# Nahuel-M/StereoVisionArray

Measured on NVIDIA B200. Metric: MDE/s, higher is better.
Workload: dtype u16

## Files before the change

stereovisionarray_b200/csrc/k_ad.cu:

```cuda
#include "sva_common.cuh"

struct AdPairs {
    int32_t alpha[SVA_MAX_PAIRS], beta[SVA_MAX_PAIRS], base[SVA_MAX_PAIRS], g[SVA_MAX_PAIRS];
    unsigned long long line_off[SVA_MAX_PAIRS];
    int32_t n;
};

__global__ void k_build_line_image(const uint8_t* __restrict__ img, int W, int H, size_t img_pitch, uint8_t* __restrict__ line,
                                   int a, int b, int u, int v, int cmin, int tmin, int pad, int pitch) {
    int x = blockIdx.x * blockDim.x + threadIdx.x, y = blockIdx.y;
    if (x >= W) return;
    int c = b * x - a * y - cmin, t = u * x + v * y - tmin + pad;
    line[(size_t)c * pitch + t] = img[(size_t)y * img_pitch + x];
}

__device__ __forceinline__ void ad_accumulate(uint32_t diff, uint32_t& even, uint32_t& odd) {
    even += diff & 0x00FF00FFu;
    odd += __byte_perm(diff, 0, 0x4341);
}

__device__ __forceinline__ void ad_gather8(const uint8_t* __restrict__ L, int off, int g, uint32_t& b0, uint32_t& b1) {
    const uint32_t* wp = (const uint32_t*)(L + (off & ~3));
    const int sh = (off & 3) * 8;
    if (g == 1) {
        uint32_t w0 = __ldg(wp), w1 = __ldg(wp + 1), w2 = __ldg(wp + 2);
        b0 = __funnelshift_r(w0, w1, sh);
        b1 = __funnelshift_r(w1, w2, sh);
    } else if (g == 2) {
        uint32_t w0 = __ldg(wp), w1 = __ldg(wp + 1), w2 = __ldg(wp + 2), w3 = __ldg(wp + 3), w4 = __ldg(wp + 4);
        uint32_t a0 = __funnelshift_r(w0, w1, sh), a1 = __funnelshift_r(w1, w2, sh);
        uint32_t a2 = __funnelshift_r(w2, w3, sh), a3 = __funnelshift_r(w3, w4, sh);
        b0 = __byte_perm(a0, a1, 0x6420);
        b1 = __byte_perm(a2, a3, 0x6420);
    } else {
        const uint8_t* q = L + off;
        b0 = q[0] | (q[g] << 8) | (q[2 * g] << 16) | ((uint32_t)q[3 * g] << 24);
        b1 = q[4 * g] | (q[5 * g] << 8) | (q[6 * g] << 16) | ((uint32_t)q[7 * g] << 24);
    }
}

__global__ void __launch_bounds__(256)
k_ad_planar(const uint8_t* __restrict__ ref, size_t ref_pitch, const uint8_t* __restrict__ lines, AdPairs P, int W, int H, int D, int dmin,
            uint32_t* __restrict__ AP, int wp, int padl, int padt) {
    const int nch = D >> 3, per_group = 2 * nch;
    const long long id = (long long)blockIdx.x * blockDim.x + threadIdx.x;
    const long long G = id / per_group;
    const int tl = (int)(id - G * per_group);
    const int half = tl / nch, chunk = tl - half * nch;
    const int tiles_x = (W + 7) >> 3;
    const long long tile = G >> 3;
    const int ty = (int)(tile / tiles_x), tx = (int)(tile - (long long)ty * tiles_x);
    const int y = ty * 8 + (int)(G & 7);
    if (y >= H) return;
    const int x0 = tx * 8 + 4 * half;
    int xc[4];
    uint32_t r4[4];
#pragma unroll
    for (int i = 0; i < 4; i++) {
        xc[i] = min(x0 + i, W - 1);
        r4[i] = (uint32_t)ref[(size_t)y * ref_pitch + xc[i]] * 0x01010101u;
    }
    const int delta0 = dmin + 8 * chunk;
    uint32_t e0[4], o0[4], e1[4], o1[4];
#pragma unroll
    for (int i = 0; i < 4; i++) { e0[i] = 0; o0[i] = 0; e1[i] = 0; o1[i] = 0; }
    for (int k = 0; k < P.n; k++) {
        const uint8_t* L = lines + P.line_off[k];
        const int g = P.g[k], alpha = P.alpha[k];
        const int offb = P.base[k] + y * P.beta[k] + g * delta0;
#pragma unroll
        for (int i = 0; i < 4; i++) {
            uint32_t b0, b1;
            ad_gather8(L, offb + xc[i] * alpha, g, b0, b1);
            ad_accumulate(__vabsdiffu4(b0, r4[i]), e0[i], o0[i]);
            ad_accumulate(__vabsdiffu4(b1, r4[i]), e1[i], o1[i]);
        }
    }
    uint32_t w[4][4];
#pragma unroll
    for (int i = 0; i < 4; i++) {
        const bool in = x0 + i < W;
        w[i][0] = in ? __byte_perm(e0[i], o0[i], 0x5410) : 0u;
        w[i][1] = in ? __byte_perm(e0[i], o0[i], 0x7632) : 0u;
        w[i][2] = in ? __byte_perm(e1[i], o1[i], 0x5410) : 0u;
        w[i][3] = in ? __byte_perm(e1[i], o1[i], 0x7632) : 0u;
    }
    uint32_t* out = AP + ((size_t)(y + padt) * (D >> 1) + 4 * chunk) * wp + padl + x0;
#pragma unroll
    for (int j = 0; j < 4; j++) *reinterpret_cast<uint4*>(out + (size_t)j * wp) = make_uint4(w[0][j], w[1][j], w[2][j], w[3][j]);
}

__global__ void k_ap_unpack(const uint32_t* __restrict__ AP, int W, int H, int dph, int wp, int padl, int padt, uint32_t* __restrict__ out) {
    const int x = blockIdx.x * blockDim.x + threadIdx.x, y = blockIdx.y;
    if (x >= W) return;
    for (int dp = 0; dp < dph; dp++) out[((size_t)y * W + x) * dph + dp] = AP[((size_t)(y + padt) * dph + dp) * wp + padl + x];
}

static void ext_gcd(int a, int b, int& g, int& u, int& v) {
    if (b == 0) { g = a < 0 ? -a : a; u = a < 0 ? -1 : 1; v = 0; return; }
    int g1, u1, v1;
    ext_gcd(b, a % b, g1, u1, v1);
    g = g1; u = v1; v = u1 - (a / b) * v1;
}

int sva_build_line_images(sva_ctx* ctx) {
    const sva_params& p = ctx->prm;
    const int W = p.width, H = p.height, dmax = p.min_disp + p.num_disp - 1;
    size_t total = 0;
    for (int k = 0; k < p.n_pairs; k++) {
        PairGeom& G = ctx->geom[k];
        int gx = p.pair_gx[k], gy = p.pair_gy[k];
        if (gx == 0 && gy == 0) return ctx->fail(SVA_ERR_BAD_ARG, "pair offset (0,0)");
        int g, u, v, one;
        ext_gcd(-gx, -gy, g, u, v);
        int a = -gx / g, b = -gy / g;
        ext_gcd(a, b, one, u, v);
        G.g = g; G.a = a; G.b = b; G.u = u; G.v = v;
        int cs[4] = {0, b * (W - 1), -a * (H - 1), b * (W - 1) - a * (H - 1)};
// ... 18 lines not shown
        const PairGeom& G = ctx->geom[k];
        dim3 grid(div_up(W, 256), H);
        LaunchScope ls(ctx, "k_build_line_image");
        k_build_line_image<<<grid, 256, 0, ctx->stream>>>(ctx->other_imgs.as<uint8_t>() + (size_t)k * W * H, W, H, (size_t)W,
                                                         ctx->lines.as<uint8_t>() + G.offset, G.a, G.b, G.u, G.v, G.cmin, G.tmin, G.pad, G.pitch);
    }
    SVA_CUDA_OK(ctx, cudaGetLastError());
    return SVA_OK;
}

int sva_ap_prepare(sva_ctx* ctx) {
    const sva_params& p = ctx->prm;
    const int W = p.width, H = p.height, D = p.num_disp, k = p.win_half;
    ApGeom g;
    const int kk = (k + 3) & ~3;
    g.padl = kk; g.padt = k;
    g.txo = (256 - kk - k + 1) & ~3;
    g.strips = div_up(W, g.txo);
    g.wp = g.txo * (g.strips - 1) + 256;
    const int need = kk + ((W + 7) & ~7);
    if (g.wp < need) g.wp = need;
    g.wp = (g.wp + 7) & ~7;
    g.hp = H + 2 * k;
    g.row_words = (size_t)(D >> 1) * g.wp;
    g.words = (size_t)g.hp * g.row_words;
    SVA_TRY(ctx->reserve(ctx->AP, g.words * 4));
    ctx->ap = g;
    uint64_t key = (uint64_t)(uintptr_t)ctx->AP.p;
    key = key * 1000003u + (uint64_t)W; key = key * 1000003u + (uint64_t)H; key = key * 1000003u + (uint64_t)D; key = key * 1000003u + (uint64_t)k;
    if (key != ctx->ap_zero_key) {
        SVA_CUDA_OK(ctx, cudaMemsetAsync(ctx->AP.p, 0, g.words * 4, ctx->stream));
        ctx->ap_zero_key = key;
    }
    return SVA_OK;
}

int sva_ap_unpack(sva_ctx* ctx) {
    const sva_params& p = ctx->prm;
    const int W = p.width, H = p.height, D = p.num_disp;
    SVA_TRY(ctx->reserve(ctx->A, (size_t)W * H * D * sizeof(uint16_t)));
    LaunchScope ls(ctx, "k_ap_unpack");
    k_ap_unpack<<<dim3(div_up(W, 128), H), 128, 0, ctx->stream>>>(ctx->AP.as<uint32_t>(), W, H, D >> 1, ctx->ap.wp, ctx->ap.padl, ctx->ap.padt, ctx->A.as<uint32_t>());
    SVA_CUDA_OK(ctx, cudaGetLastError());
    return SVA_OK;
}

int sva_run_ad(sva_ctx* ctx) {
    const sva_params& p = ctx->prm;
    const int W = p.width, H = p.height, D = p.num_disp;
    SVA_TRY(sva_ap_prepare(ctx));
    AdPairs P;
    P.n = ctx->pair_end - ctx->pair_begin;
    for (int i = 0; i < P.n; i++) {
        const PairGeom& G = ctx->geom[ctx->pair_begin + i];
        P.alpha[i] = G.alpha; P.beta[i] = G.beta; P.base[i] = G.base; P.g[i] = G.g; P.line_off[i] = G.offset;
    }
    {
        LaunchScope ls(ctx, "k_ad_planar");
        const long long threads = (long long)div_up(W, 8) * div_up(H, 8) * 8 * (2 * (D >> 3));
        k_ad_planar<<<(unsigned)((threads + 255) / 256), 256, 0, ctx->stream>>>(ctx->ref_img.as<uint8_t>(), (size_t)W, ctx->lines.as<uint8_t>(), P, W, H, D, p.min_disp,
                                                                             ctx->AP.as<uint32_t>(), ctx->ap.wp, ctx->ap.padl, ctx->ap.padt);
    }
    SVA_CUDA_OK(ctx, cudaGetLastError());
    ctx->have_ad = true;
    return SVA_OK;
}
```

stereovisionarray_b200/csrc/k_ad2.cu:

```cuda
#include <algorithm>
#include <cstdlib>

#include "sva_common.cuh"

#define AD2_TH 8
#define AD2_TW 128
#define AD2_DR 32
#define AD2_THREADS 512
#define AD2_MAXG 2
#define AD2_SMEM_BUDGET (110 * 1024)

__host__ __device__ constexpr int ad2_sp(int agx, int dr = AD2_DR) { return dr == 32 ? (agx == 0 ? 160 : (agx == 1 ? 192 : 224)) : (agx == 0 ? 160 : (agx == 1 ? 176 : 192)); }
__host__ __device__ constexpr int ad2_rows(int agy, int th, int dr = AD2_DR) { return th + (dr - 1) * agy; }
#define AD2_TH_MAX 48

struct Ad2Params {
    const uint8_t* ref;
    const uint8_t* imgs;
    size_t img_bytes;
    int rp, pp, padx, pady;
    int W, H, D, dmin;
    uint32_t* AP;
    int wp, padl, padt;
    int n;
    int8_t gx[SVA_MAX_PAIRS], gy[SVA_MAX_PAIRS], phi[SVA_MAX_PAIRS];
    uint8_t img[SVA_MAX_PAIRS];
    int ngroups;
    uint8_t gbeg[SVA_MAX_PAIRS + 1];
    int row0, row1;
    int th;
    uint32_t one;
};

template <int GX, int GY, bool FMA = false, int DR = AD2_DR>
__device__ __forceinline__ void ad2_pair(const uint32_t* __restrict__ bp, const uint32_t r, uint32_t (&ax)[16], uint32_t (&ao)[16], const uint32_t one = 1u) {
    constexpr int SP = ad2_sp(GX < 0 ? -GX : GX, DR);
#pragma unroll
    for (int i = 0; i < 16; i++) {
        const int boff = -i * (GY * SP + GX);
        const int al = ((boff % 4) + 4) % 4;
        const int w0 = (boff - al) / 4;
        uint32_t w = bp[w0];
        if (al != 0) w = __funnelshift_r(w, bp[w0 + 1], 8 * al);
        const uint32_t ad = __vabsdiffu4(w, r);
        if (FMA) {
            ax[i] = ad * one + ax[i];
// ... 67 lines not shown
        sh.src[k] = q.imgs + (size_t)q.img[k] * q.img_bytes + (size_t)(q.pady + ylo) * q.pp + c0;
        sh.geo[k] = make_int2(soff, rows);
    }
    __syncthreads();
    const uint32_t smem_base = (uint32_t)__cvta_generic_to_shared(smem);
    for (int k = kb; k < ke; k++) {
        const int2 geo = sh.geo[k];
        const int sp = sh.pk[k].y, cpr = sp >> 4, n = geo.y * cpr;
        const uint32_t inv = 65536u / (uint32_t)cpr + 1u;
        const uint8_t* src0 = sh.src[k];
        const uint32_t dst0 = smem_base + geo.x;
        for (int c = t; c < n; c += AD2_THREADS) {
            const int rr = (int)(((uint32_t)c * inv) >> 16), cc = (c - rr * cpr) << 4;
            asm volatile("cp.async.cg.shared.global [%0], [%1], 16;" ::"r"(dst0 + rr * sp + cc), "l"(src0 + (size_t)rr * q.pp + cc) : "memory");
        }
    }
    asm volatile("cp.async.commit_group;" ::: "memory");
    asm volatile("cp.async.wait_group 0;" ::: "memory");
    __syncthreads();
}

__device__ __forceinline__ void ad2_store(const Ad2Params& q, const int y, const int x, const int d0, const uint32_t (&ax)[16], const uint32_t (&ao)[16]) {
    if (y >= q.H || x >= q.W || d0 >= q.D) return;
    uint32_t* out = q.AP + ((size_t)(y + q.padt) * (q.D >> 1) + (d0 >> 1)) * q.wp + q.padl + x;
    uint32_t me = 0xFFFFFFFFu, mo = 0xFFFFFFFFu;
    if (x + 3 >= q.W) {
        me = (x + 2 < q.W) ? 0xFFFFFFFFu : 0x0000FFFFu;
        mo = (x + 1 < q.W) ? 0x0000FFFFu : 0u;
    }
    const int np = min(8, (q.D - d0) >> 1);
#pragma unroll
    for (int i = 0; i < 8; i++) {
        const uint32_t o0 = ao[2 * i] & mo, o1 = ao[2 * i + 1] & mo;
        const uint32_t e0 = (ax[2 * i] - (ao[2 * i] << 8)) & me, e1 = (ax[2 * i + 1] - (ao[2 * i + 1] << 8)) & me;
        const uint4 v = make_uint4(__byte_perm(e0, e1, 0x5410), __byte_perm(o0, o1, 0x5410), __byte_perm(e0, e1, 0x7632), __byte_perm(o0, o1, 0x7632));
        if (i < np) *reinterpret_cast<uint4*>(out + (size_t)i * q.wp) = v;
    }
}

template <bool MULTI>
__global__ void __launch_bounds__(AD2_THREADS, 2)
k_ad_tile(const Ad2Params q) {
    extern __shared__ __align__(16) unsigned char ad2_smem[];
    __shared__ Ad2Shared sh;
    const int t = threadIdx.x;
    const int quad = t & 31, sub = (t >> 5) & 1, yl = t >> 6;
    const int x0 = blockIdx.x * AD2_TW, y0 = q.row0 + blockIdx.y * q.th, da = blockIdx.z * AD2_DR;
    const int x = x0 + 4 * quad, d0 = da + 16 * sub;
    uint32_t ax[16], ao[16];
    if (MULTI) {
        const int y = y0 + yl;
        const uint32_t r = *reinterpret_cast<const uint32_t*>(q.ref + (size_t)y * q.rp + x);
#pragma unroll
        for (int i = 0; i < 16; i++) { ax[i] = 0; ao[i] = 0; }
        for (int g = 0; g < q.ngroups; g++) {
            const int kb = q.gbeg[g], ke = q.gbeg[g + 1];
            if (g > 0) __syncthreads();
            ad2_stage(q, sh, ad2_smem, kb, ke, x0, y0, da);
#pragma unroll 1
// ... 121 lines not shown
        SVA_CUDA_OK(ctx, cudaMemsetAsync(ctx->pad_ref.p, 0, (size_t)g.rp * g.ref_rows, ctx->stream));
        ctx->ad2_zero_key = key;
    }
    ctx->ad2 = g;
    return SVA_OK;
}

uint8_t* sva_ad2_view_origin(sva_ctx* ctx, int k) {
    const sva_params& p = ctx->prm;
    const int phi = ((p.pair_gx[k] * p.min_disp) % 4 + 4) % 4;
    return ctx->pad_imgs.as<uint8_t>() + (size_t)k * ctx->ad2.img_bytes + (size_t)ctx->ad2.pady * ctx->ad2.pp + ctx->ad2.padx + phi;
}

int sva_ap_prepare(sva_ctx* ctx);

int sva_run_ad2(sva_ctx* ctx) {
    const sva_params& p = ctx->prm;
    const int W = p.width, H = p.height, D = p.num_disp;
    SVA_TRY(sva_ap_prepare(ctx));
    Ad2Params q{};
    q.ref = ctx->pad_ref.as<uint8_t>(); q.imgs = ctx->pad_imgs.as<uint8_t>(); q.img_bytes = ctx->ad2.img_bytes;
    q.rp = ctx->ad2.rp; q.pp = ctx->ad2.pp; q.padx = ctx->ad2.padx; q.pady = ctx->ad2.pady;
    q.W = W; q.H = H; q.D = D; q.dmin = p.min_disp;
    q.AP = ctx->AP.as<uint32_t>(); q.wp = ctx->ap.wp; q.padl = ctx->ap.padl; q.padt = ctx->ap.padt;
    q.n = ctx->pair_end - ctx->pair_begin;
    q.one = 1u;
    for (int i = 0; i < q.n; i++) {
        const int k = ctx->pair_begin + i;
        q.gx[i] = (int8_t)p.pair_gx[k]; q.gy[i] = (int8_t)p.pair_gy[k]; q.img[i] = (uint8_t)k;
        q.phi[i] = (int8_t)(((p.pair_gx[k] * p.min_disp) % 4 + 4) % 4);
    }
    if (q.n == 0) {
        SVA_CUDA_OK(ctx, cudaMemsetAsync(ctx->AP.p, 0, ctx->ap.words * 4, ctx->stream));
        ctx->have_ad = true;
        return SVA_OK;
    }
    int ya = 0, yb = H;
    if (ctx->win_rows > 0) { ya = std::max(0, ctx->win_y0 - p.win_half); yb = std::min(H, ctx->win_y0 + ctx->win_rows + p.win_half); }
    q.row0 = ya / AD2_TH * AD2_TH; q.row1 = yb;
    void (*kern)(Ad2Params) = nullptr;
    int dr = AD2_DR;
    if (ctx->tune_ad_set) {
        if (ad2_set_matches<Ad2Set3x3>(q)) { kern = k_ad_tile_set<Ad2Set3x3>; dr = Ad2Set3x3::dr; }
        else if (ad2_set_matches<Ad2SetPair>(q)) { kern = k_ad_tile_set<Ad2SetPair>; dr = Ad2SetPair::dr; }
        else if (ad2_set_matches<Ad2Set4x4>(q)) { kern = k_ad_tile_set<Ad2Set4x4>; dr = Ad2Set4x4::dr; }
    }
    const int rstep = dr == 32 ? 8 : 16;
// ... 40 lines not shown
```

stereovisionarray_b200/csrc/k_box.cu:

```cuda
#include <algorithm>

#include "sva_common.cuh"

#define BOX_THREADS 256
#define BOX_DP 16
#define BOX_CG 16
#define BOX_MAX_BAND 512

struct BoxParams {
    const uint16_t* A;
    void* out;
    int W, H, D, k, dmin, shift, cap;
    int gxp, gxn, gyp, gyn;
    int band_rows, txo;
    int apply_validity;
};

__device__ __forceinline__ int axis_limit(int pos, int dim, int k, int gp, int gn) {
    if (pos < k || pos >= dim - k) return -1;
    int lim = 0x7FFFFFFF;
    if (gp > 0) lim = min(lim, (pos - k) / gp);
    if (gn > 0) lim = min(lim, (dim - k - pos) / gn);
    return lim;
}
// ... 142 lines not shown
    if (bands < 1) bands = 1;
    if (div_up(H, bands) > BOX_MAX_BAND) bands = div_up(H, BOX_MAX_BAND);
    q.band_rows = div_up(H, bands);
    bands = div_up(H, q.band_rows);
    dim3 grid(strips, dch, bands);
    LaunchScope ls(ctx, raw ? "k_box_cost_raw" : "k_box_cost");
    cudaError_t e;
    if (wide) e = raw ? box_launch<8, true>(q, grid, ctx->stream) : box_launch<8, false>(q, grid, ctx->stream);
    else e = raw ? box_launch<4, true>(q, grid, ctx->stream) : box_launch<4, false>(q, grid, ctx->stream);
    SVA_CUDA_OK(ctx, e);
    return SVA_OK;
}

#define BXP_WARPS 8
#define BXP_TCOLS 48
#define BXP_OPITCH 260
#define BXP_MAX_BAND 1024

struct BoxPParams {
    const uint32_t* AP;
    uint16_t* C;
    int W, H, D, k, kk, dmin, shift, cap;
    int gxp, gxn, gyp, gyn;
    int band_rows, txo, wp;
    int l2hint;
    int chunk;
    long long row_words;
    int ry0, ry1;
};

__global__ void __launch_bounds__(256, 2)
k_box_planar(BoxPParams q) {
    __shared__ __align__(16) uint32_t s_out[2][BXP_WARPS][BXP_OPITCH];
    __shared__ __align__(8) unsigned long long s_bar[2];
    __shared__ uint2 s_T[BXP_WARPS][8 * BXP_TCOLS];
    __shared__ int s_limy[BXP_MAX_BAND];
    const int t = threadIdx.x, lane = t & 31, warp = t >> 5;
    const int W = q.W, H = q.H, D = q.D, k = q.k;
    const int dpc = min((int)blockIdx.y * BXP_WARPS + warp, (D >> 1) - 1);
    const int d = 2 * dpc;
    const int xs = blockIdx.x * q.txo - q.kk;
    const int y0 = q.ry0 + blockIdx.z * q.band_rows, y1 = min(q.ry1, y0 + q.band_rows);
    for (int i = t; i < y1 - y0; i += 256) s_limy[i] = axis_limit(y0 + i, H, k, q.gyp, q.gyn);

    int thr[8], thrmin = 0x7FFFFFFF;
#pragma unroll
    for (int j = 0; j < 8; j++) {
        thr[j] = axis_limit(xs + lane * 8 + j, W, k, q.gxp, q.gxn) - q.dmin - d;
        thrmin = min(thrmin, thr[j]);
    }
    uint2* tbl = &s_T[warp][8 + lane];
    if (lane == 0) tbl[0] = make_uint2(0u, 0u);
    const uint32_t bar0 = (uint32_t)__cvta_generic_to_shared(&s_bar[0]);
    if (t == 0) {
        asm volatile("mbarrier.init.shared::cta.b64 [%0], %1;" ::"r"(bar0), "r"(BXP_WARPS) : "memory");
        asm volatile("mbarrier.init.shared::cta.b64 [%0], %1;" ::"r"(bar0 + 8), "r"(BXP_WARPS) : "memory");
    }
    int offh[8], offl[8];
#pragma unroll
    for (int j = 0; j < 8; j++) {
        offh[j] = ((j + k) & 7) * BXP_TCOLS + ((j + k) >> 3);
        offl[j] = ((j - k) & 7) * BXP_TCOLS + ((j - k) >> 3);
    }
    __syncthreads();

    const uint32_t* pz = q.AP + (size_t)dpc * q.wp + (size_t)blockIdx.x * q.txo + lane * 8;
    const uint32_t* pe = pz + (size_t)y0 * q.row_words;
    const long long back = 2LL * k * q.row_words;
    const int N = (y1 - y0) + 2 * k - 1;
    uint32_t F[8], Vh[8];
#pragma unroll
    for (int j = 0; j < 8; j++) { F[j] = 0; Vh[j] = 0; }

    const int hf = t & 1;
    const bool half_ok = (int)blockIdx.y * 16 + 8 * hf < D;
    const int xl0 = t >> 1, xl1 = xl0 + 128;
    const bool st0 = half_ok && xl0 >= q.kk && xl0 < q.kk + q.txo && xs + xl0 < W;
    const bool st1 = half_ok && xl1 >= q.kk && xl1 < q.kk + q.txo && xs + xl1 < W;
    uint16_t* po = q.C + ((size_t)y0 * W + (xs + xl0)) * D + blockIdx.y * 16 + 8 * hf;
    const size_t orow = (size_t)W * D;
    const uint32_t kB = (uint32_t)k << 16;

    auto store_row = [&](const int r) {
        const uint32_t bar = bar0 + 8 * (r & 1), parity = (uint32_t)(r >> 1) & 1u;
        asm volatile(
            "{\n"
            ".reg .pred p;\n"
            "BOXWAIT_%=:\n"
            "mbarrier.try_wait.parity.shared::cta.b64 p, [%0], %1;\n"
            "@p bra BOXDONE_%=;\n"
            "bra BOXWAIT_%=;\n"
// ... 50 lines not shown
            for (int j = 0; j < 8; j++) {
                const uint2 hi = tbl[offh[j]], lo = tbl[offl[j]];
                const uint32_t chi = hi.y - lo.y - B;
                const uint32_t clo = hi.x - lo.x - B2 - (chi << 16);
                uint32_t c0 = min(clo >> q.shift, (uint32_t)q.cap), c1 = min(chi >> q.shift, (uint32_t)q.cap);
                const int m = min(thr[j], srow);
                c0 = m >= 0 ? c0 : (uint32_t)q.cap;
                c1 = m >= 1 ? c1 : (uint32_t)q.cap;
                w[j] = c1 * 65536u + c0;
            }
        }
        if (it > 0) store_row(it - 1);
        uint32_t* so = &s_out[it & 1][warp][lane * 8];
        *reinterpret_cast<uint4*>(so) = make_uint4(w[0], w[1], w[2], w[3]);
        *reinterpret_cast<uint4*>(so + 4) = make_uint4(w[4], w[5], w[6], w[7]);
        __syncwarp();
        if (lane == 0) asm volatile("mbarrier.arrive.shared::cta.b64 _, [%0];" ::"r"(bar0 + 8 * (it & 1)) : "memory");
    };

    uint4 a0 = ldg_stream_u128(pe), a1 = ldg_stream_u128(pe + 4), al0 = make_uint4(0, 0, 0, 0), al1 = al0;
    uint4 b0 = a0, b1 = a1, bl0 = al0, bl1 = al1;
    auto fetch = [&](const int n, uint4& e0, uint4& e1, uint4& l0, uint4& l1) {
        if (n < N) {
            pe += q.row_words;
            const uint32_t* pl = n >= 2 * k ? pe - back : pz;
            e0 = ldg_stream_u128(pe); e1 = ldg_stream_u128(pe + 4);
            l0 = ldg_stream_u128(pl); l1 = ldg_stream_u128(pl + 4);
        }
    };
    for (int n = 0; n < N; n += 2) {
        fetch(n + 1, b0, b1, bl0, bl1);
        row(n, a0, a1, al0, al1);
        if (n + 1 >= N) break;
        fetch(n + 2, a0, a1, al0, al1);
        row(n + 1, b0, b1, bl0, bl1);
    }
    store_row(y1 - y0 - 1);
}

template <int K, int PF, int OCC>
__global__ void __launch_bounds__(256, OCC)
k_box_planar_shfl(BoxPParams q) {
    static_assert(K % 8 == 4 && K >= 4 && K <= 56, "window half-width must be 4 mod 8");
    constexpr int M = (K - 4) / 8;
    __shared__ __align__(16) uint32_t s_out[2][BXP_WARPS][BXP_OPITCH];
    __shared__ __align__(8) unsigned long long s_bar[2];
    __shared__ int s_limy[BXP_MAX_BAND];
    const int t = threadIdx.x, lane = t & 31, warp = t >> 5;
    const int W = q.W, H = q.H, D = q.D;
    const int dpc = min((int)blockIdx.y * BXP_WARPS + warp, (D >> 1) - 1);
    const int d = 2 * dpc;
    const int xs = blockIdx.x * q.txo - K;
    const int y0 = q.ry0 + blockIdx.z * q.band_rows, y1 = min(q.ry1, y0 + q.band_rows);
    for (int i = t; i < y1 - y0; i += 256) s_limy[i] = axis_limit(y0 + i, H, K, q.gyp, q.gyn);

    int thr[8], thrmin = 0x7FFFFFFF;
#pragma unroll
    for (int j = 0; j < 8; j++) {
        thr[j] = axis_limit(xs + lane * 8 + j, W, K, q.gxp, q.gxn) - q.dmin - d;
        thrmin = min(thrmin, thr[j]);
    }
    const uint32_t bar0 = (uint32_t)__cvta_generic_to_shared(&s_bar[0]);
    if (t == 0) {
        asm volatile("mbarrier.init.shared::cta.b64 [%0], %1;" ::"r"(bar0), "r"(BXP_WARPS) : "memory");
        asm volatile("mbarrier.init.shared::cta.b64 [%0], %1;" ::"r"(bar0 + 8), "r"(BXP_WARPS) : "memory");
    }
    __syncthreads();

    const unsigned long long pol_enter = q.l2hint ? l2_policy_evict_last() : l2_policy_evict_normal();
    const unsigned long long pol_leave = q.l2hint ? l2_policy_evict_first() : l2_policy_evict_normal();
    const uint32_t* pe = q.AP + (size_t)dpc * q.wp + (size_t)blockIdx.x * q.txo + lane * 8 + (size_t)y0 * q.row_words;
    const long long back = 2LL * K * q.row_words;
    const int N = (y1 - y0) + 2 * K - 1;
    uint32_t F[8], Hh[8];
#pragma unroll
    for (int j = 0; j < 8; j++) { F[j] = 0; Hh[j] = 0; }

    const int hf = t & 1;
    const bool half_ok = (int)blockIdx.y * 16 + 8 * hf < D;
    const int xl0 = t >> 1, xl1 = xl0 + 128;
    const bool st0 = half_ok && xl0 >= K && xl0 < K + q.txo && xs + xl0 < W;
    const bool st1 = half_ok && xl1 >= K && xl1 < K + q.txo && xs + xl1 < W;
    uint16_t* po = q.C + ((size_t)y0 * W + (xs + xl0)) * D + blockIdx.y * 16 + 8 * hf;
    const size_t orow = (size_t)W * D;

    auto store_row = [&](const int r) {
        const uint32_t bar = bar0 + 8 * (r & 1), parity = (uint32_t)(r >> 1) & 1u;
        asm volatile(
            "{\n"
            ".reg .pred p;\n"
            "BOXSWAIT_%=:\n"
            "mbarrier.try_wait.parity.shared::cta.b64 p, [%0], %1;\n"
            "@p bra BOXSDONE_%=;\n"
            "bra BOXSWAIT_%=;\n"
            "BOXSDONE_%=:\n"
// ... 49 lines not shown
                const int m = min(thr[j], srow);
                c0 = m >= 0 ? c0 : (uint32_t)q.cap;
                c1 = m >= 1 ? c1 : (uint32_t)q.cap;
                w[j] = c1 * 65536u + c0;
            }
        }
        if (it > 0) store_row(it - 1);
        uint32_t* so = &s_out[it & 1][warp][lane * 8];
        const bool swz = (lane & 4) != 0;
        *reinterpret_cast<uint4*>(so + (swz ? 4 : 0)) = swz ? make_uint4(w[4], w[5], w[6], w[7]) : make_uint4(w[0], w[1], w[2], w[3]);
        *reinterpret_cast<uint4*>(so + (swz ? 0 : 4)) = swz ? make_uint4(w[0], w[1], w[2], w[3]) : make_uint4(w[4], w[5], w[6], w[7]);
        __syncwarp();
        if (lane == 0) asm volatile("mbarrier.arrive.shared::cta.b64 _, [%0];" ::"r"(bar0 + 8 * (it & 1)) : "memory");
    };

    {
        uint32_t acc[8];
#pragma unroll
        for (int j = 0; j < 8; j++) acc[j] = 0x80008000u;
        int cnt = 0;
        U32x8 a = ldg_stream_u256(pe, pol_enter);
        for (int n = 0; n < 2 * K - 1; n++) {
            U32x8 b = a;
            if (n + 1 < 2 * K - 1) { pe += q.row_words; b = ldg_stream_u256(pe, pol_enter); }
#pragma unroll
            for (int j = 0; j < 8; j++) acc[j] += a.v[j];
            if (++cnt == q.chunk || n + 1 == 2 * K - 1) {
                hpass(acc);
#pragma unroll
                for (int j = 0; j < 8; j++) acc[j] = 0x80008000u;
                cnt = 0;
            }
            a = b;
        }
    }
    {
        const int R = y1 - y0;
        auto fetch = [&](const int it, U32x8& e, U32x8& l) {
            if (it < R) {
                pe += q.row_words;
                e = ldg_stream_u256(pe, pol_enter);
                if (it > 0) l = ldg_stream_u256(pe - back, pol_leave);
            }
        };
        auto row = [&](const int it, const U32x8& e, const U32x8& l) {
            uint32_t u[8];
#pragma unroll
            for (int j = 0; j < 8; j++) u[j] = e.v[j] - l.v[j] + 0x80008000u;
            hpass(u);
            emit(it);
        };
        U32x8 be[PF + 1], bl[PF + 1];
#pragma unroll
        for (int i = 0; i <= PF; i++)
#pragma unroll
            for (int j = 0; j < 8; j++) { be[i].v[j] = 0; bl[i].v[j] = 0; }
#pragma unroll
        for (int i = 0; i < PF; i++) fetch(i, be[i], bl[i]);
        for (int it = 0; it < R; it += PF + 1) {
#pragma unroll
            for (int i = 0; i <= PF; i++) {
                if (it + i < R) {
                    fetch(it + i + PF, be[(i + PF) % (PF + 1)], bl[(i + PF) % (PF + 1)]);
// ... 2 lines not shown
            }
        }
        store_row(R - 1);
    }
    (void)N;
}

int sva_ap_prepare(sva_ctx* ctx);
int sva_ap_unpack(sva_ctx* ctx);

static int sva_launch_box_planar(sva_ctx* ctx) {
    const sva_params& p = ctx->prm;
    const int W = p.width, H = p.height, D = p.num_disp, k = p.win_half;
    BoxPParams q{};
    q.AP = ctx->AP.as<uint32_t>(); q.C = ctx->C.as<uint16_t>();
    q.W = W; q.H = H; q.D = D; q.k = k; q.kk = ctx->ap.padl; q.dmin = p.min_disp; q.shift = p.cost_shift; q.cap = p.cost_cap;
    for (int i = 0; i < p.n_pairs; i++) {
        int gx = p.pair_gx[i], gy = p.pair_gy[i];
        if (gx > 0) q.gxp = gx > q.gxp ? gx : q.gxp;
        if (gx < 0) q.gxn = -gx > q.gxn ? -gx : q.gxn;
        if (gy > 0) q.gyp = gy > q.gyp ? gy : q.gyp;
        if (gy < 0) q.gyn = -gy > q.gyn ? -gy : q.gyn;
    }
    q.txo = ctx->ap.txo; q.wp = ctx->ap.wp; q.row_words = (long long)ctx->ap.row_words;
    const int strips = ctx->ap.strips, dgroups = div_up(D, 16);
    const bool shfl = ctx->tune_box_shfl && k % 8 == 4;
    auto shfl_kernel = [&](int occ) -> void (*)(BoxPParams) {
        switch (k) {
            case 4: return occ == 3 ? k_box_planar_shfl<4, 1, 3> : k_box_planar_shfl<4, 1, 2>;
            case 12: return occ == 3 ? k_box_planar_shfl<12, 1, 3> : k_box_planar_shfl<12, 1, 2>;
            case 20: return occ == 3 ? k_box_planar_shfl<20, 1, 3> : k_box_planar_shfl<20, 1, 2>;
            case 28: return occ == 3 ? k_box_planar_shfl<28, 1, 3> : k_box_planar_shfl<28, 1, 2>;
            case 36: return occ == 3 ? k_box_planar_shfl<36, 1, 3> : k_box_planar_shfl<36, 1, 2>;
            case 44: return occ == 3 ? k_box_planar_shfl<44, 1, 3> : k_box_planar_shfl<44, 1, 2>;
            default: return occ == 3 ? k_box_planar_shfl<52, 1, 3> : k_box_planar_shfl<52, 1, 2>;
        }
    };
    if (shfl) {
        q.chunk = std::max(1, 32767 / (255 * p.n_pairs));
        q.l2hint = ctx->tune_box_l2 ? 1 : 0;
    }
    q.ry0 = 0; q.ry1 = H;
    if (ctx->win_rows > 0) { q.ry0 = ctx->win_y0; q.ry1 = ctx->win_y0 + ctx->win_rows; }
    const int Hw = q.ry1 - q.ry0;
    void (*kern)(BoxPParams) = k_box_planar;
    const char* label = shfl ? "k_box_planar_shfl" : "k_box_planar";
    int bands = 1;
// ... 43 lines not shown
```

stereovisionarray_b200/csrc/k_census.cu:

```cuda
#include "sva_common.cuh"

#define CENSUS_RX 4
#define CENSUS_RY 3

__global__ void __launch_bounds__(128)
k_census_transform(const uint8_t* __restrict__ img, size_t pitch, int W, int H, uint64_t* __restrict__ out) {
    const int x = blockIdx.x * 128 + threadIdx.x, y = blockIdx.y;
    if (x >= W) return;
    const int c = img[(size_t)y * pitch + x];
    uint64_t t = 0;
    int bit = 0;
#pragma unroll
    for (int dy = -CENSUS_RY; dy <= CENSUS_RY; dy++) {
        const int yy = y + dy;
        const bool row_ok = yy >= 0 && yy < H;
#pragma unroll
        for (int dx = -CENSUS_RX; dx <= CENSUS_RX; dx++) {
            if (dx == 0 && dy == 0) continue;
            const int xx = x + dx;
            const int v = (row_ok && xx >= 0 && xx < W) ? (int)__ldg(img + (size_t)yy * pitch + xx) : 0;
            t |= (uint64_t)(v < c) << bit;
            bit++;
        }
    }
    out[(size_t)y * W + x] = t;
}

struct CensusPairs {
    int n;
    int gx[SVA_MAX_PAIRS], gy[SVA_MAX_PAIRS];
    int view[SVA_MAX_PAIRS];
};

__global__ void __launch_bounds__(128)
k_ad_census(const uint64_t* __restrict__ tr, const uint64_t* __restrict__ to, const CensusPairs P, int W, int H, int D, int dmin,
            uint32_t* __restrict__ AP, int wp, int padl, int padt) {
    const int x = blockIdx.x * 128 + threadIdx.x, y = blockIdx.y, d0 = blockIdx.z * 8;
    if (x >= W) return;
    const uint64_t r = tr[(size_t)y * W + x];
    uint32_t acc[8];
#pragma unroll
    for (int i = 0; i < 8; i++) acc[i] = 0;
    const size_t px = (size_t)W * H;
    for (int k = 0; k < P.n; k++) {
        const uint64_t* t = to + px * P.view[k];
        const int gx = P.gx[k], gy = P.gy[k];
#pragma unroll
        for (int i = 0; i < 8; i++) {
            const int delta = dmin + d0 + i, sx = x - gx * delta, sy = y - gy * delta;
            uint64_t v = 0;
            if (sx >= 0 && sx < W && sy >= 0 && sy < H) v = __ldg(t + (size_t)sy * W + sx);
            acc[i] += __popcll(r ^ v);
        }
    }
    uint32_t* out = AP + ((size_t)(y + padt) * (D >> 1) + (d0 >> 1)) * wp + padl + x;
#pragma unroll
    for (int i = 0; i < 4; i++)
        if (d0 + 2 * i < D) out[(size_t)i * wp] = acc[2 * i] | (acc[2 * i + 1] << 16);
}

int sva_ap_prepare(sva_ctx* ctx);

int sva_run_ad_census(sva_ctx* ctx) {
    const sva_params& p = ctx->prm;
    const int W = p.width, H = p.height, D = p.num_disp;
    const size_t px = (size_t)W * H;
    SVA_TRY(sva_ap_prepare(ctx));
    SVA_TRY(ctx->reserve(ctx->census, px * sizeof(uint64_t) * (size_t)(p.n_pairs + 1)));
    uint64_t* tr = ctx->census.as<uint64_t>();
    uint64_t* to = tr + px;
    const dim3 g2(div_up(W, 128), H);
    {
        LaunchScope ls(ctx, "k_census_transform");
        k_census_transform<<<g2, 128, 0, ctx->stream>>>(ctx->ref_img.as<uint8_t>(), (size_t)W, W, H, tr);
        for (int i = ctx->pair_begin; i < ctx->pair_end; i++)
            k_census_transform<<<g2, 128, 0, ctx->stream>>>(ctx->other_imgs.as<uint8_t>() + px * i, (size_t)W, W, H, to + px * i);
        ctx->launches += ctx->pair_end - ctx->pair_begin;
    }
    SVA_CUDA_OK(ctx, cudaGetLastError());
    CensusPairs P{};
    P.n = ctx->pair_end - ctx->pair_begin;
    for (int i = 0; i < P.n; i++) { P.gx[i] = p.pair_gx[ctx->pair_begin + i]; P.gy[i] = p.pair_gy[ctx->pair_begin + i]; P.view[i] = ctx->pair_begin + i; }
    {
        LaunchScope ls(ctx, "k_ad_census");
        k_ad_census<<<dim3(div_up(W, 128), H, div_up(D, 8)), 128, 0, ctx->stream>>>(tr, to, P, W, H, D, p.min_disp, ctx->AP.as<uint32_t>(), ctx->ap.wp, ctx->ap.padl, ctx->ap.padt);
    }
    SVA_CUDA_OK(ctx, cudaGetLastError());
    ctx->have_ad = true;
    return SVA_OK;
}
```

stereovisionarray_b200/csrc/sva_common.cuh:

```cuda
#pragma once
#include <cuda_runtime.h>
#include <stdint.h>

#include <set>
#include <string>
#include <vector>

#include "../../include/sva_c_api.h"

#define SVA_CUDA_OK(ctx, expr)                                                                         \
    do {                                                                                               \
        cudaError_t e__ = (expr);                                                                      \
        if (e__ != cudaSuccess) return (ctx)->fail(SVA_ERR_CUDA, std::string(#expr) + ": " + cudaGetErrorString(e__)); \
    } while (0)

#define SVA_TRY(expr)            \
    do {                         \
        int rc__ = (expr);       \
        if (rc__ != SVA_OK) return rc__; \
    } while (0)

struct DevBuf {
    void* p = nullptr;
    size_t bytes = 0;
    void* base = nullptr;
    template <typename T> T* as() const { return (T*)p; }
};

struct PairGeom {
    int32_t alpha, beta, base;
    int32_t g;
    int32_t rows, pitch;
    int32_t a, b, u, v, cmin, tmin, pad;
    size_t offset;
};

struct ApGeom {
    int wp = 0, hp = 0, padl = 0, padt = 0;
    int txo = 0, strips = 0;
    size_t row_words = 0, words = 0;
};

struct Ad2Geom {
    int padx = 0, pady = 0, pp = 0, rows = 0;
    int rp = 0, ref_rows = 0;
    size_t img_bytes = 0;
};

struct IoSet {
    DevBuf pad_ref, pad_imgs, ref_img, other_imgs, lines, mask, disp, subpix;
    uint64_t ad2_zero_key = 0;
};

struct KernelTime {
    const char* name;
    cudaEvent_t beg, end;
};

struct sva_ctx {
    int device = 0;
    int sm_count = 148;
    cudaStream_t own_stream = nullptr;
    cudaStream_t stream = nullptr;
    cudaStream_t aux_stream = nullptr;
// ... 11 lines not shown
    std::string err;
    uint64_t launches = 0;

    bool have_frame = false, have_ad = false, have_cost = false, have_sgm = false, have_disp = false;
    sva_params prm{};
    sva_params up_prm{};
    bool ad_params_ok = false;
    int ad_y0 = 0, ad_y1 = 0, cost_y0 = 0, cost_y1 = 0;
    int pair_begin = 0, pair_end = 0;
    bool has_mask = false;
    bool debug_store_full_s = false;
    int tune_sgm_split = 1;
    int tune_sgm_hstore = 2;
    int tune_sgm_pace = -1;
    int tune_sgm_pace_window = 2;
    int tune_sgm_bulk = 0;
    int tune_sgm_diag_split = 1;
    int tune_ad_gather = 0;
    int tune_ad_set = 1;
    int tune_ad_th = 0;
    int tune_box_l2 = 0;
    int tune_box_occ = 0;
    int tune_box_bands = 0;
    int tune_box_shfl = 1;
    int tune_wta_seg = -1;
    uint32_t sgm_dir_mask_override = 0;
    PairGeom geom[SVA_MAX_PAIRS];
    DevBuf ref_img, other_imgs, lines, mask, A, AP, C, Craw, S, disp, subpix, other_d, scratch, scratch2, pace_buf;
    DevBuf pad_imgs, pad_ref, comm_scratch, census, tex_img, sgm_state;
    unsigned long long tex = 0;
    uint64_t tex_key = 0;
    void* comm = nullptr;
    int comm_rank = 0, comm_world = 1;
    void* rows_link = nullptr;
    Ad2Geom ad2;
    uint64_t ad2_zero_key = 0;
    bool use_ad2 = false;
    ApGeom ap;
    uint64_t ap_zero_key = 0;
    DevBuf staging_host;
    int win_y0 = 0, win_rows = 0;
    bool guard = false;
    void device_bufs(std::vector<DevBuf*>& out);
    void release(DevBuf& b);

    bool timing = false;
// ... 73 lines not shown
```

stereovisionarray_b200/csrc/sva_ctx.cu:

```cuda
#include <cstdio>
#include <cstdlib>

#include "sva_common.cuh"

void sva_dist_release(sva_ctx* c);

static constexpr size_t GUARD_BYTES = 256 << 10;
static constexpr int GUARD_CANARY = 0xA5, GUARD_POISON = 0xCD;

__global__ void k_guard_count(const uint8_t* __restrict__ p, size_t n, unsigned long long* bad) {
    unsigned long long local = 0;
    for (size_t i = blockIdx.x * (size_t)blockDim.x + threadIdx.x; i < n; i += (size_t)gridDim.x * blockDim.x) local += p[i] != GUARD_CANARY;
    if (local) atomicAdd(bad, local);
}

void sva_ctx::release(DevBuf& b) {
    if (b.p) cudaFree(b.base ? b.base : b.p);
    b.p = b.base = nullptr;
    b.bytes = 0;
}

void sva_ctx::device_bufs(std::vector<DevBuf*>& out) {
    out = {&ref_img, &other_imgs, &lines, &mask, &A, &AP, &pad_imgs, &pad_ref, &C, &Craw, &S, &disp, &subpix, &other_d, &scratch, &scratch2, &pace_buf, &comm_scratch, &census, &tex_img, &sgm_state,
           &alt.pad_ref, &alt.pad_imgs, &alt.ref_img, &alt.other_imgs, &alt.lines, &alt.mask, &alt.disp, &alt.subpix};
// ... 55 lines not shown
    *out = nullptr;
    int n = 0;
    if (cudaGetDeviceCount(&n) != cudaSuccess || n <= 0 || device < 0 || device >= n) return SVA_ERR_NO_DEVICE;
    cudaDeviceProp prop;
    if (cudaGetDeviceProperties(&prop, device) != cudaSuccess) return SVA_ERR_CUDA;
    if (prop.major != 10) return SVA_ERR_NO_DEVICE;
    if (cudaSetDevice(device) != cudaSuccess) return SVA_ERR_CUDA;
    sva_ctx* c = new sva_ctx();
    c->device = device;
    c->sm_count = prop.multiProcessorCount;
    if (cudaStreamCreateWithFlags(&c->own_stream, cudaStreamNonBlocking) != cudaSuccess) { delete c; return SVA_ERR_CUDA; }
    c->stream = c->own_stream;
    if (const char* e = getenv("SVA_SGM_SPLIT")) c->tune_sgm_split = atoi(e);
    if (const char* e = getenv("SVA_SGM_PACE")) c->tune_sgm_pace = atoi(e);
    if (const char* e = getenv("SVA_SGM_HSTORE")) c->tune_sgm_hstore = atoi(e);
    if (const char* e = getenv("SVA_STREAM_AD_AHEAD")) c->tune_stream_ad_ahead = atoi(e);
    if (const char* e = getenv("SVA_SGM_BULK")) c->tune_sgm_bulk = atoi(e);
    if (const char* e = getenv("SVA_PREZERO")) c->tune_prezero = atoi(e);
    if (const char* e = getenv("SVA_SGM_DIAG_SPLIT")) c->tune_sgm_diag_split = atoi(e);
    if (const char* e = getenv("SVA_WTA_SEG")) c->tune_wta_seg = atoi(e);
    if (const char* e = getenv("SVA_AD_GATHER")) c->tune_ad_gather = atoi(e);
    if (const char* e = getenv("SVA_AD_TH")) c->tune_ad_th = atoi(e);
    if (const char* e = getenv("SVA_BOX_SHFL")) c->tune_box_shfl = atoi(e);
    if (const char* e = getenv("SVA_BOX_L2")) c->tune_box_l2 = atoi(e);
    if (const char* e = getenv("SVA_BOX_BANDS")) c->tune_box_bands = atoi(e);
    if (const char* e = getenv("SVA_BOX_OCC")) c->tune_box_occ = atoi(e);
    if (const char* e = getenv("SVA_AD_SET")) c->tune_ad_set = atoi(e);
    if (const char* e = getenv("SVA_SGM_PACE_WINDOW")) c->tune_sgm_pace_window = atoi(e);
    *out = c;
    return SVA_OK;
}

int sva_destroy(sva_ctx* c) {
    if (!c) return SVA_ERR_BAD_ARG;
    cudaSetDevice(c->device);
    if (c->stream == c->own_stream) cudaStreamSynchronize(c->stream);
    else cudaDeviceSynchronize();
    sva_dist_release(c);
    if (c->tex) cudaDestroyTextureObject((cudaTextureObject_t)c->tex);
    if (c->aux_stream) cudaStreamSynchronize(c->aux_stream);
    if (c->h2d_stream) { cudaStreamSynchronize(c->h2d_stream); cudaStreamSynchronize(c->d2h_stream); }
    if (c->ad_stream) cudaStreamSynchronize(c->ad_stream);
    std::vector<DevBuf*> bufs;
    c->device_bufs(bufs);
    for (DevBuf* b : bufs) c->release(*b);
    if (c->h2d_stream) {
// ... 81 lines not shown
```

Before: 130,800.

## Tile the AP cost volume by box-filter strips with duplicated overlap columns

Changes the packed AD cost volume from a row-major plane-per-disparity layout to a layout tiled by box-filter strips and groups of 8 disparity planes, with each strip 256 words wide. Producers write into every tile that covers a column, duplicating the overlap region. The box filter then reads each strip as a contiguous block with a short row stride, which should improve DRAM/L2 locality and TLB behaviour. In exchange it adds extra duplicate writes, more index arithmetic, and a larger buffer. The tiled layout is on by default behind an env toggle.

```diff
diff --git a/stereovisionarray_b200/csrc/k_ad.cu b/stereovisionarray_b200/csrc/k_ad.cu
--- a/stereovisionarray_b200/csrc/k_ad.cu
+++ b/stereovisionarray_b200/csrc/k_ad.cu
@@ -41,7 +41,7 @@
 
 __global__ void __launch_bounds__(256)
 k_ad_planar(const uint8_t* __restrict__ ref, size_t ref_pitch, const uint8_t* __restrict__ lines, AdPairs P, int W, int H, int D, int dmin,
-            uint32_t* __restrict__ AP, int wp, int padl, int padt) {
+            uint32_t* __restrict__ AP, const ApGeom ag) {
     const int nch = D >> 3, per_group = 2 * nch;
     const long long id = (long long)blockIdx.x * blockDim.x + threadIdx.x;
     const long long G = id / per_group;
@@ -85,15 +85,22 @@
         w[i][2] = in ? __byte_perm(e1[i], o1[i], 0x5410) : 0u;
         w[i][3] = in ? __byte_perm(e1[i], o1[i], 0x7632) : 0u;
     }
-    uint32_t* out = AP + ((size_t)(y + padt) * (D >> 1) + 4 * chunk) * wp + padl + x0;
-#pragma unroll
-    for (int j = 0; j < 4; j++) *reinterpret_cast<uint4*>(out + (size_t)j * wp) = make_uint4(w[0][j], w[1][j], w[2][j], w[3][j]);
-}
-
-__global__ void k_ap_unpack(const uint32_t* __restrict__ AP, int W, int H, int dph, int wp, int padl, int padt, uint32_t* __restrict__ out) {
+    const int pc = ag.padl + x0;
+    int t0, t1;
+    ap_tiles_of(ag, pc, t0, t1);
+    for (int t = t0; t <= t1; t++) {
+        uint32_t* out = AP + ap_word_index(ag.ix, y + ag.padt, 4 * chunk, pc, t);
+#pragma unroll
+        for (int j = 0; j < 4; j++) *reinterpret_cast<uint4*>(out + (size_t)j * ag.ix.plane_words) = make_uint4(w[0][j], w[1][j], w[2][j], w[3][j]);
+    }
+}
+
+__global__ void k_ap_unpack(const uint32_t* __restrict__ AP, int W, int H, int dph, const ApGeom ag, uint32_t* __restrict__ out) {
     const int x = blockIdx.x * blockDim.x + threadIdx.x, y = blockIdx.y;
     if (x >= W) return;
-    for (int dp = 0; dp < dph; dp++) out[((size_t)y * W + x) * dph + dp] = AP[((size_t)(y + padt) * dph + dp) * wp + padl + x];
+    int t0, t1;
+    ap_tiles_of(ag, ag.padl + x, t0, t1);
+    for (int dp = 0; dp < dph; dp++) out[((size_t)y * W + x) * dph + dp] = AP[ap_word_index(ag.ix, y + ag.padt, dp, ag.padl + x, t1)];
 }
 
 static void ext_gcd(int a, int b, int& g, int& u, int& v) {
@@ -158,12 +165,26 @@
     if (g.wp < need) g.wp = need;
     g.wp = (g.wp + 7) & ~7;
     g.hp = H + 2 * k;
-    g.row_words = (size_t)(D >> 1) * g.wp;
-    g.words = (size_t)g.hp * g.row_words;
+    g.tiled = ctx->tune_ap_tiled ? 1 : 0;
+    ApIndex& x = g.ix;
+    if (g.tiled) {
+        x.tile_x = g.txo;
+        x.plane_words = 256;
+        x.row_words = 8 * 256;
+        x.tile_words = (size_t)g.hp * x.row_words;
+        x.group_words = (size_t)g.strips * x.tile_words;
+        g.words = (size_t)div_up(D, 16) * x.group_words;
+    } else {
+        x.plane_words = g.wp;
+        x.row_words = (size_t)(D >> 1) * g.wp;
+        x.group_words = 8 * (size_t)g.wp;
+        g.words = (size_t)g.hp * x.row_words;
+    }
     SVA_TRY(ctx->reserve(ctx->AP, g.words * 4));
     ctx->ap = g;
     uint64_t key = (uint64_t)(uintptr_t)ctx->AP.p;
     key = key * 1000003u + (uint64_t)W; key = key * 1000003u + (uint64_t)H; key = key * 1000003u + (uint64_t)D; key = key * 1000003u + (uint64_t)k;
+    key = key * 1000003u + (uint64_t)g.tiled;
     if (key != ctx->ap_zero_key) {
         SVA_CUDA_OK(ctx, cudaMemsetAsync(ctx->AP.p, 0, g.words * 4, ctx->stream));
         ctx->ap_zero_key = key;
@@ -176,7 +197,7 @@
     const int W = p.width, H = p.height, D = p.num_disp;
     SVA_TRY(ctx->reserve(ctx->A, (size_t)W * H * D * sizeof(uint16_t)));
     LaunchScope ls(ctx, "k_ap_unpack");
-    k_ap_unpack<<<dim3(div_up(W, 128), H), 128, 0, ctx->stream>>>(ctx->AP.as<uint32_t>(), W, H, D >> 1, ctx->ap.wp, ctx->ap.padl, ctx->ap.padt, ctx->A.as<uint32_t>());
+    k_ap_unpack<<<dim3(div_up(W, 128), H), 128, 0, ctx->stream>>>(ctx->AP.as<uint32_t>(), W, H, D >> 1, ctx->ap, ctx->A.as<uint32_t>());
     SVA_CUDA_OK(ctx, cudaGetLastError());
     return SVA_OK;
 }
@@ -195,7 +216,7 @@
         LaunchScope ls(ctx, "k_ad_planar");
         const long long threads = (long long)div_up(W, 8) * div_up(H, 8) * 8 * (2 * (D >> 3));
         k_ad_planar<<<(unsigned)((threads + 255) / 256), 256, 0, ctx->stream>>>(ctx->ref_img.as<uint8_t>(), (size_t)W, ctx->lines.as<uint8_t>(), P, W, H, D, p.min_disp,
-                                                                             ctx->AP.as<uint32_t>(), ctx->ap.wp, ctx->ap.padl, ctx->ap.padt);
+                                                                             ctx->AP.as<uint32_t>(), ctx->ap);
     }
     SVA_CUDA_OK(ctx, cudaGetLastError());
     ctx->have_ad = true;
diff --git a/stereovisionarray_b200/csrc/k_ad2.cu b/stereovisionarray_b200/csrc/k_ad2.cu
--- a/stereovisionarray_b200/csrc/k_ad2.cu
+++ b/stereovisionarray_b200/csrc/k_ad2.cu
@@ -21,7 +21,7 @@
     int rp, pp, padx, pady;
     int W, H, D, dmin;
     uint32_t* AP;
-    int wp, padl, padt;
+    ApGeom ag;
     int n;
     int8_t gx[SVA_MAX_PAIRS], gy[SVA_MAX_PAIRS], phi[SVA_MAX_PAIRS];
     uint8_t img[SVA_MAX_PAIRS];
@@ -135,7 +135,12 @@
 
 __device__ __forceinline__ void ad2_store(const Ad2Params& q, const int y, const int x, const int d0, const uint32_t (&ax)[16], const uint32_t (&ao)[16]) {
     if (y >= q.H || x >= q.W || d0 >= q.D) return;
-    uint32_t* out = q.AP + ((size_t)(y + q.padt) * (q.D >> 1) + (d0 >> 1)) * q.wp + q.padl + x;
+    const int pc = q.ag.padl + x;
+    int t0, t1;
+    ap_tiles_of(q.ag, pc, t0, t1);
+    uint32_t* out = q.AP + ap_word_index(q.ag.ix, y + q.ag.padt, d0 >> 1, pc, t1);
+    const size_t pw = q.ag.ix.plane_words, dup = (size_t)(t1 - t0) * (q.ag.ix.tile_words - q.ag.ix.tile_x);
+    const bool two = t0 < t1;
     uint32_t me = 0xFFFFFFFFu, mo = 0xFFFFFFFFu;
     if (x + 3 >= q.W) {
         me = (x + 2 < q.W) ? 0xFFFFFFFFu : 0x0000FFFFu;
@@ -147,7 +152,10 @@
         const uint32_t o0 = ao[2 * i] & mo, o1 = ao[2 * i + 1] & mo;
         const uint32_t e0 = (ax[2 * i] - (ao[2 * i] << 8)) & me, e1 = (ax[2 * i + 1] - (ao[2 * i + 1] << 8)) & me;
         const uint4 v = make_uint4(__byte_perm(e0, e1, 0x5410), __byte_perm(o0, o1, 0x5410), __byte_perm(e0, e1, 0x7632), __byte_perm(o0, o1, 0x7632));
-        if (i < np) *reinterpret_cast<uint4*>(out + (size_t)i * q.wp) = v;
+        if (i < np) {
+            *reinterpret_cast<uint4*>(out + (size_t)i * pw) = v;
+            if (two) *reinterpret_cast<uint4*>(out + (size_t)i * pw - dup) = v;
+        }
     }
 }
 
@@ -315,7 +323,7 @@
     q.ref = ctx->pad_ref.as<uint8_t>(); q.imgs = ctx->pad_imgs.as<uint8_t>(); q.img_bytes = ctx->ad2.img_bytes;
     q.rp = ctx->ad2.rp; q.pp = ctx->ad2.pp; q.padx = ctx->ad2.padx; q.pady = ctx->ad2.pady;
     q.W = W; q.H = H; q.D = D; q.dmin = p.min_disp;
-    q.AP = ctx->AP.as<uint32_t>(); q.wp = ctx->ap.wp; q.padl = ctx->ap.padl; q.padt = ctx->ap.padt;
+    q.AP = ctx->AP.as<uint32_t>(); q.ag = ctx->ap;
     q.n = ctx->pair_end - ctx->pair_begin;
     q.one = 1u;
     for (int i = 0; i < q.n; i++) {
diff --git a/stereovisionarray_b200/csrc/k_box.cu b/stereovisionarray_b200/csrc/k_box.cu
--- a/stereovisionarray_b200/csrc/k_box.cu
+++ b/stereovisionarray_b200/csrc/k_box.cu
@@ -188,10 +188,10 @@
     uint16_t* C;
     int W, H, D, k, kk, dmin, shift, cap;
     int gxp, gxn, gyp, gyn;
-    int band_rows, txo, wp;
+    int band_rows, txo;
     int l2hint;
     int chunk;
-    long long row_words;
+    ApIndex ax;
     int ry0, ry1;
 };
 
@@ -230,9 +230,9 @@
     }
     __syncthreads();
 
-    const uint32_t* pz = q.AP + (size_t)dpc * q.wp + (size_t)blockIdx.x * q.txo + lane * 8;
-    const uint32_t* pe = pz + (size_t)y0 * q.row_words;
-    const long long back = 2LL * k * q.row_words;
+    const uint32_t* pz = q.AP + ap_word_index(q.ax, 0, dpc, blockIdx.x * q.txo + lane * 8, q.ax.tile_x ? blockIdx.x : 0);
+    const uint32_t* pe = pz + (size_t)y0 * q.ax.row_words;
+    const long long back = 2LL * k * q.ax.row_words;
     const int N = (y1 - y0) + 2 * k - 1;
     uint32_t F[8], Vh[8];
 #pragma unroll
@@ -329,7 +329,7 @@
     uint4 b0 = a0, b1 = a1, bl0 = al0, bl1 = al1;
     auto fetch = [&](const int n, uint4& e0, uint4& e1, uint4& l0, uint4& l1) {
         if (n < N) {
-            pe += q.row_words;
+            pe += q.ax.row_words;
             const uint32_t* pl = n >= 2 * k ? pe - back : pz;
             e0 = ldg_stream_u128(pe); e1 = ldg_stream_u128(pe + 4);
             l0 = ldg_stream_u128(pl); l1 = ldg_stream_u128(pl + 4);
@@ -376,8 +376,8 @@
 
     const unsigned long long pol_enter = q.l2hint ? l2_policy_evict_last() : l2_policy_evict_normal();
     const unsigned long long pol_leave = q.l2hint ? l2_policy_evict_first() : l2_policy_evict_normal();
-    const uint32_t* pe = q.AP + (size_t)dpc * q.wp + (size_t)blockIdx.x * q.txo + lane * 8 + (size_t)y0 * q.row_words;
-    const long long back = 2LL * K * q.row_words;
+    const uint32_t* pe = q.AP + ap_word_index(q.ax, y0, dpc, blockIdx.x * q.txo + lane * 8, q.ax.tile_x ? blockIdx.x : 0);
+    const long long back = 2LL * K * q.ax.row_words;
     const int N = (y1 - y0) + 2 * K - 1;
     uint32_t F[8], Hh[8];
 #pragma unroll
@@ -473,7 +473,7 @@
         U32x8 a = ldg_stream_u256(pe, pol_enter);
         for (int n = 0; n < 2 * K - 1; n++) {
             U32x8 b = a;
-            if (n + 1 < 2 * K - 1) { pe += q.row_words; b = ldg_stream_u256(pe, pol_enter); }
+            if (n + 1 < 2 * K - 1) { pe += q.ax.row_words; b = ldg_stream_u256(pe, pol_enter); }
 #pragma unroll
             for (int j = 0; j < 8; j++) acc[j] += a.v[j];
             if (++cnt == q.chunk || n + 1 == 2 * K - 1) {
@@ -489,7 +489,7 @@
         const int R = y1 - y0;
         auto fetch = [&](const int it, U32x8& e, U32x8& l) {
             if (it < R) {
-                pe += q.row_words;
+                pe += q.ax.row_words;
                 e = ldg_stream_u256(pe, pol_enter);
                 if (it > 0) l = ldg_stream_u256(pe - back, pol_leave);
             }
@@ -538,7 +538,7 @@
         if (gy > 0) q.gyp = gy > q.gyp ? gy : q.gyp;
         if (gy < 0) q.gyn = -gy > q.gyn ? -gy : q.gyn;
     }
-    q.txo = ctx->ap.txo; q.wp = ctx->ap.wp; q.row_words = (long long)ctx->ap.row_words;
+    q.txo = ctx->ap.txo; q.ax = ctx->ap.ix;
     const int strips = ctx->ap.strips, dgroups = div_up(D, 16);
     const bool shfl = ctx->tune_box_shfl && k % 8 == 4;
     auto shfl_kernel = [&](int occ) -> void (*)(BoxPParams) {
diff --git a/stereovisionarray_b200/csrc/k_census.cu b/stereovisionarray_b200/csrc/k_census.cu
--- a/stereovisionarray_b200/csrc/k_census.cu
+++ b/stereovisionarray_b200/csrc/k_census.cu
@@ -34,7 +34,7 @@
 
 __global__ void __launch_bounds__(128)
 k_ad_census(const uint64_t* __restrict__ tr, const uint64_t* __restrict__ to, const CensusPairs P, int W, int H, int D, int dmin,
-            uint32_t* __restrict__ AP, int wp, int padl, int padt) {
+            uint32_t* __restrict__ AP, const ApGeom ag) {
     const int x = blockIdx.x * 128 + threadIdx.x, y = blockIdx.y, d0 = blockIdx.z * 8;
     if (x >= W) return;
     const uint64_t r = tr[(size_t)y * W + x];
@@ -53,10 +53,15 @@
             acc[i] += __popcll(r ^ v);
         }
     }
-    uint32_t* out = AP + ((size_t)(y + padt) * (D >> 1) + (d0 >> 1)) * wp + padl + x;
+    const int pc = ag.padl + x;
+    int t0, t1;
+    ap_tiles_of(ag, pc, t0, t1);
+    for (int t = t0; t <= t1; t++) {
+        uint32_t* out = AP + ap_word_index(ag.ix, y + ag.padt, d0 >> 1, pc, t);
 #pragma unroll
-    for (int i = 0; i < 4; i++)
-        if (d0 + 2 * i < D) out[(size_t)i * wp] = acc[2 * i] | (acc[2 * i + 1] << 16);
+        for (int i = 0; i < 4; i++)
+            if (d0 + 2 * i < D) out[(size_t)i * ag.ix.plane_words] = acc[2 * i] | (acc[2 * i + 1] << 16);
+    }
 }
 
 int sva_ap_prepare(sva_ctx* ctx);
@@ -83,7 +88,7 @@
     for (int i = 0; i < P.n; i++) { P.gx[i] = p.pair_gx[ctx->pair_begin + i]; P.gy[i] = p.pair_gy[ctx->pair_begin + i]; P.view[i] = ctx->pair_begin + i; }
     {
         LaunchScope ls(ctx, "k_ad_census");
-        k_ad_census<<<dim3(div_up(W, 128), H, div_up(D, 8)), 128, 0, ctx->stream>>>(tr, to, P, W, H, D, p.min_disp, ctx->AP.as<uint32_t>(), ctx->ap.wp, ctx->ap.padl, ctx->ap.padt);
+        k_ad_census<<<dim3(div_up(W, 128), H, div_up(D, 8)), 128, 0, ctx->stream>>>(tr, to, P, W, H, D, p.min_disp, ctx->AP.as<uint32_t>(), ctx->ap);
     }
     SVA_CUDA_OK(ctx, cudaGetLastError());
     ctx->have_ad = true;
diff --git a/stereovisionarray_b200/csrc/sva_common.cuh b/stereovisionarray_b200/csrc/sva_common.cuh
--- a/stereovisionarray_b200/csrc/sva_common.cuh
+++ b/stereovisionarray_b200/csrc/sva_common.cuh
@@ -35,11 +35,29 @@
     size_t offset;
 };
 
+struct ApIndex {
+    size_t group_words = 0, tile_words = 0, row_words = 0;
+    int plane_words = 0;
+    int tile_x = 0;
+};
 struct ApGeom {
     int wp = 0, hp = 0, padl = 0, padt = 0;
     int txo = 0, strips = 0;
-    size_t row_words = 0, words = 0;
-};
+    int tiled = 0;
+    ApIndex ix;
+    size_t words = 0;
+};
+
+__host__ __device__ __forceinline__ size_t ap_word_index(const ApIndex& g, int row, int plane, int pc, int t) {
+    return (size_t)(plane >> 3) * g.group_words + (size_t)t * g.tile_words + (size_t)row * g.row_words + (size_t)(plane & 7) * g.plane_words +
+           (size_t)(pc - t * g.tile_x);
+}
+__host__ __device__ __forceinline__ void ap_tiles_of(const ApGeom& g, int pc, int& t0, int& t1) {
+    if (!g.tiled) { t0 = t1 = 0; return; }
+    t1 = min(pc / g.txo, g.strips - 1);
+    t0 = (t1 > 0 && pc < (t1 - 1) * g.txo + 256) ? t1 - 1 : t1;
+    if (pc >= t1 * g.txo + 256) t0 = t1 + 1;
+}
 
 struct Ad2Geom {
     int padx = 0, pady = 0, pp = 0, rows = 0;
@@ -97,6 +115,7 @@
     int tune_box_l2 = 0;
     int tune_box_occ = 0;
     int tune_box_bands = 0;
+    int tune_ap_tiled = 1;
     int tune_box_shfl = 1;
     int tune_wta_seg = -1;
     uint32_t sgm_dir_mask_override = 0;
diff --git a/stereovisionarray_b200/csrc/sva_ctx.cu b/stereovisionarray_b200/csrc/sva_ctx.cu
--- a/stereovisionarray_b200/csrc/sva_ctx.cu
+++ b/stereovisionarray_b200/csrc/sva_ctx.cu
@@ -101,6 +101,7 @@
     if (const char* e = getenv("SVA_AD_GATHER")) c->tune_ad_gather = atoi(e);
     if (const char* e = getenv("SVA_AD_TH")) c->tune_ad_th = atoi(e);
     if (const char* e = getenv("SVA_BOX_SHFL")) c->tune_box_shfl = atoi(e);
+    if (const char* e = getenv("SVA_AP_TILED")) c->tune_ap_tiled = atoi(e);
     if (const char* e = getenv("SVA_BOX_L2")) c->tune_box_l2 = atoi(e);
     if (const char* e = getenv("SVA_BOX_BANDS")) c->tune_box_bands = atoi(e);
     if (const char* e = getenv("SVA_BOX_OCC")) c->tune_box_occ = atoi(e);
```

New measurement: 130,100, median of 6. No clear change (-0.5%).
